# kfkq/DQMC

Hardware: AMD Instinct MI355X
Metric: MC sweeps/sec, 2D Hubbard N=256 Ltau=200 (higher is better)
Workload: dtype f64; 1 GPU; cfg3: 16x16 Hubbard U=8.0 beta=8.0 Ltau=200 n_stab=10 t=1 mu=-0.1; chains_per_gpu=1, n_chains_total=1, parallelism=independent chains, 1 gpu x 1 chain

## Files before the change

dqmc_amd/csrc/common.h:

```cpp
#pragma once

#include <hip/hip_runtime.h>
#include <cstdint>
#include <memory>
#include <string>

struct dqmc_engine;

namespace dq {

constexpr int WAVE = 64;

void set_error(const std::string& msg);
const char* get_error();

#define DQ_HIP(call)                                                                    \
    do {                                                                                \
        hipError_t _e = (call);                                                         \
        if (_e != hipSuccess) {                                                         \
            ::dq::set_error(std::string(#call) + ": " + hipGetErrorString(_e));         \
            return -2;                                              \
        }                                                                               \
    } while (0)

// ... 20 lines not shown

struct Mat {
    double* p = nullptr;
    long stride = 0;
    __host__ __device__ double* at(int c) const { return p + (long)c * stride; }
};
struct CMat {
    const double* p = nullptr;
    long stride = 0;
    CMat() = default;
    __host__ __device__ CMat(const double* p_, long s) : p(p_), stride(s) {}
    __host__ __device__ CMat(const Mat& m) : p(m.p), stride(m.stride) {}
    __host__ __device__ const double* at(int c) const { return p + (long)c * stride; }
};
using Vec = Mat;
using CVec = CMat;

struct GemmDesc {
    CMat A, B;
    Mat C;
    Mat CT{nullptr, 0};
    CVec rs, ks, cs;
    int n = 0;
    int transA = 0;
    int accumulate = 0;
};
int launch_gemm(const GemmDesc& g, int n_chains, hipStream_t s);

int launch_build_expv(const int8_t* fields, long f_stride, int nt, int n, const double* tab_expv ,
                      double* expv, double* invexpv, long v_stride, int n_chains, hipStream_t s);
int launch_split_d(CVec d, Vec dl_inv, Vec ds, double* logsum, int n, int n_chains, hipStream_t s);
int launch_split_d2(CVec d1, Vec dl1, Vec ds1, CVec d2, Vec dl2, Vec ds2, int n, int n_chains, hipStream_t s);
int launch_measure_equal_time(CMat G, double* out, long out_stride, int L1, int L2, int accumulate, int n_chains, hipStream_t s);
int launch_measure_unequal_time(const double* Gtt, const double* Gt0, const double* G0t, double* out, long out_stride, int L1, int L2, int nt,
                                int accumulate, int n_chains, hipStream_t s);
int launch_axpb_identity(CMat in, Mat out, double a, double b, int n, int n_chains, hipStream_t s);
int launch_copy(CMat in, Mat out, long count, int n_chains, hipStream_t s);
int launch_set_identity(Mat out, int n, int n_chains, hipStream_t s);
int launch_transpose_scale(CMat in, Mat out, CVec rs, int n, int n_chains, hipStream_t s);
int launch_max_abs_diff(CMat A, CMat B, double* err, long err_stride, int n, int n_chains, hipStream_t s);
int launch_add_scaled_cols(CMat A, CMat B, CVec cs, Mat C, int n, int n_chains, hipStream_t s);
int launch_scale_rows(CMat in, CVec rs, Mat out, int n, int n_chains, hipStream_t s);
struct DevStats { double acc_rate, max_err, sum_err, n_err; long long n_accepted, n_proposed; };
int launch_fold_stats(DevStats* st, const int* acc, long acc_stride, int n_slices, const double* err, long err_stride, int n_err,
                      int n, int nt, int n_chains, hipStream_t s);

struct QrWork {
    double* tau; long tau_stride;
    int* jpvt; long jpvt_stride;
    unsigned long long* sync = nullptr; long sync_stride = 0;
    int* abort_words = nullptr;
    int* info = nullptr;
    double* pw = nullptr; long pw_stride = 0;
    int* pivpos = nullptr; long pivpos_stride = 0;
};
long qr_panel_work_doubles(int n);
int launch_qr_panel(Mat A, Mat L, QrWork w, int n, int n_chains, hipStream_t s);
long qrcp_coop_sync_granules(int n);
int qrcp_coop_workgroups(int n, int n_chains);
enum class QrFamily { Panel, ColumnOwner, Cooperative, Streaming };
int launch_to_ldr(QrFamily f, Mat A, Mat L, Vec d, Mat R, QrWork w, int n, int n_chains, hipStream_t s);

int launch_lu_blocked(Mat A, int* perm, long perm_stride, int* rowpos, long rowpos_stride, double* logabsdet, int accumulate_logdet,
                      int* info, int n, int n_chains, hipStream_t s);
int launch_lu_solve(CMat LU, const int* perm, long perm_stride, Mat X, CVec dg, int mode, int n, int n_chains, hipStream_t s);

int launch_tri_solve(CMat R, const int* perm, long perm_stride, Mat X, CVec dg, double* scratch, long scratch_stride, int n, int n_chains, hipStream_t s);

int launch_gj_solve(Mat A, Mat B, Mat X, Mat SA, double* tinv, int* perm, long perm_stride, int* rowpos, long rowpos_stride,
                    double* logabsdet, int accumulate_logdet, int* info, int n, int n_chains, hipStream_t s);

struct UpdateTables {
    double rb[4][3];
    double delta[4][3];
    double ev[4];
    double iev[4];
    double pad[32];
};
struct UpdateDesc {
    Mat G;
    int8_t* fields; long f_stride;
    double* expv; double* invexpv; long v_stride;
    const UpdateTables* tabs;
    const int32_t* perm; const uint8_t* kprop; const double* u; long rs_stride;
    double* Upanel; double* Wpanel; long panel_stride;
    double* Cpanel = nullptr;
    int* state; long state_stride;
    double* prep; long prep_stride;
    Mat GT{nullptr, 0};
    int gt_valid = 0;
    void* slice_sync = nullptr;
    unsigned slice_epoch = 0;
    int slice_absent_tile = -1;
    int slice_absent_l = -1;
    int slice_late_tile = -1, slice_late_us = 0;
    int* info = nullptr;
    int* acc_out; long acc_stride;
    int n, nt;
};
constexpr int UPDATE_KD = 32;

struct SliceSync {
    unsigned long long seq; unsigned int error; unsigned int solo_count; unsigned int pad[12];
    unsigned int arrive[496];
};
constexpr size_t SLICE_SYNC_BYTES = 2048;
static_assert(sizeof(SliceSync) == SLICE_SYNC_BYTES, "SliceSync layout");
constexpr unsigned SLICE_EPOCH_LIMIT = 1u << 24;
constexpr unsigned SLICE_SOLO_BIT = 1u << 30, SLICE_FINAL_BIT = 1u << 31;
// ... 36 lines not shown
```

dqmc_amd/csrc/engine.hip:

```cpp
#include "common.h"
#include "../../include/dqmc_hip.h"

#include <cmath>
#include <cstdlib>
#include <cstring>
#include <map>
#include <memory>
#include <mutex>
#include <vector>

namespace dq {

static thread_local std::string g_err;
void set_error(const std::string& msg) { g_err = msg; }
const char* get_error() { return g_err.c_str(); }

int init_device_kernels(int device) {
    static std::mutex mu; static bool done[64] = {};
    std::lock_guard<std::mutex> lk(mu);
    if (device < 0 || device >= 64) { set_error("device ordinal out of range"); return -1; }
    if (done[device]) return 0;
    DQ_HIP(hipSetDevice(device));
    DQ_TRY(update_init_device()); DQ_TRY(update_sm_init_device()); DQ_TRY(qr_init_device()); DQ_TRY(qr_colown_init_device());
    done[device] = true;
    return 0;
}

struct Switches { bool qr_panel, qr_streaming, walk_submatrix, lu_classic, slice_multikernel; };
static const Switches& switches() {
    static const Switches sw = [] {
        const char* panel = getenv("DQMC_QR_PANEL");
        return Switches{!(panel && atoi(panel) == 0), getenv("DQMC_QR_STREAMING") != nullptr, getenv("DQMC_WALK_SUBMATRIX") != nullptr,
                        getenv("DQMC_LU_CLASSIC") != nullptr, getenv("DQMC_SLICE_MULTIKERNEL") != nullptr};
    }();
    return sw;
}

constexpr int GJ_MAX_N = 1024, GJ_MAX_CHAINS = 8;
constexpr int TRI_MAX_N = 640;

static QrFamily pick_qr(int n, int chains, bool allow_panel) {
    const Switches& sw = switches();
    if (sw.qr_streaming) return QrFamily::Streaming;
    if (allow_panel && sw.qr_panel && n >= 64 && n <= 1024 && n % 16 == 0 && chains <= 8) return QrFamily::Panel;
    if (n <= 256) return QrFamily::ColumnOwner;
    return qrcp_coop_workgroups(n, chains) <= 200 ? QrFamily::Cooperative : QrFamily::Streaming;
}

struct KernelPlan {
    QrFamily qr;
    enum class Solve { GaussJordan, BlockedLu } solve;
    enum class Rinv { Blocked, PerColumn } rinv;
    static KernelPlan pick(int n, int chains) {
        return KernelPlan{pick_qr(n, chains, true),
                          n <= GJ_MAX_N && chains <= GJ_MAX_CHAINS && !switches().lu_classic ? Solve::GaussJordan : Solve::BlockedLu,
                          n <= TRI_MAX_N ? Rinv::Blocked : Rinv::PerColumn};
    }
};

static SlicePath pick_slice_path(int n, int chains, bool reserved) {
    const Switches& sw = switches();
    const bool walk = n <= 256;
    if (sw.slice_multikernel) return SlicePath::Pairs;
    if (reserved) return walk && !sw.walk_submatrix ? SlicePath::PersistentWalk : SlicePath::PersistentSubmatrix;
    if (!walk) return SlicePath::Pairs;
    return chains >= 224 ? SlicePath::Solo : SlicePath::PairsTailSolo;
}
static bool is_persistent(SlicePath p) { return p == SlicePath::PersistentWalk || p == SlicePath::PersistentSubmatrix; }

struct LdrRef {
    Mat L; Vec d; Mat R;
    int* jpvt = nullptr;
    bool* tri = nullptr;
    Mat X{nullptr, 0};
    bool* xok = nullptr;
    void touch() const { if (xok) *xok = false; }
};
struct LdrStore {
    int n = 0, C = 0;
    DevPtr<double> L, d, R, X;
    DevPtr<int> jpvt;
    std::unique_ptr<bool[]> tri, xok;
    int alloc(int k, int n_, int C_, bool with_x = false) {
        n = n_; C = C_;
        const size_t nn = (size_t)n * n;
        DQ_TRY(dev_alloc(L, (size_t)k * C * nn)); DQ_TRY(dev_alloc(d, (size_t)k * C * n));
        DQ_TRY(dev_alloc(R, (size_t)k * C * nn)); DQ_TRY(dev_alloc(jpvt, (size_t)k * C * n));
        if (with_x) DQ_TRY(dev_alloc(X, (size_t)k * C * nn));
        tri.reset(new bool[k]()); xok.reset(new bool[k]());
        return 0;
    }
    LdrRef at(int i) const {
        const long nn = (long)n * n;
        LdrRef f{Mat{L.get() + (long)i * C * nn, nn}, Vec{d.get() + (long)i * C * n, (long)n}, Mat{R.get() + (long)i * C * nn, nn},
                 jpvt.get() + (long)i * C * n, &tri[i]};
        if (X) { f.X = Mat{X.get() + (long)i * C * nn, nn}; f.xok = &xok[i]; }
        return f;
    }
};

struct Ctx {
    int n = 0, C = 0, device = 0;
    long nn = 0;
    hipStream_t stream = nullptr;
    static constexpr int NT = 6, NV = 5;
    DevPtr<double> pool;
    DevPtr<double> vpool;
    DevPtr<int> ipool;
    DevPtr<unsigned long long> qsync;
    DevPtr<int> qabort;
    DevPtr<double> tinv;
    DevPtr<double> qpw;
    DevPtr<int> qpivpos;
    DevPtr<double> trinv;
    KernelPlan plan{};

    Mat T(int k) const { return Mat{pool.get() + (long)k * C * nn, nn}; }
    Vec V(int k) const { return Vec{vpool.get() + (long)k * C * n, (long)n}; }
    int* jpvt() const { return ipool.get(); }
    int* lperm() const { return ipool.get() + (long)C * n; }
    int* rowpos() const { return ipool.get() + 2L * C * n; }
    int* info() const { return ipool.get() + 3L * C * n; }

    int init(int n_, int C_, int device_) {
        n = n_; C = C_; device = device_; nn = (long)n * n;
        DQ_HIP(hipSetDevice(device));
        DQ_TRY(init_device_kernels(device));
        DQ_HIP(hipStreamCreateWithFlags(&stream, hipStreamNonBlocking));
        DQ_TRY(dev_alloc(pool, (size_t)NT * C * nn));
        DQ_TRY(dev_alloc(vpool, (size_t)NV * C * n));
        DQ_TRY(dev_alloc(ipool, 3L * C * n + 4));
        plan = KernelPlan::pick(n, C);
        if (plan.qr == QrFamily::Cooperative) { DQ_TRY(dev_alloc(qsync, (size_t)qrcp_coop_sync_granules(n) * C)); DQ_TRY(dev_alloc(qabort, C)); }
        if (plan.qr == QrFamily::Panel) { DQ_TRY(dev_alloc(qpw, (size_t)qr_panel_work_doubles(n) * C)); DQ_TRY(dev_alloc(qpivpos, (size_t)n * C)); }
        if (plan.solve == KernelPlan::Solve::GaussJordan) DQ_TRY(dev_alloc(tinv, (size_t)2048 * C));
        if (plan.rinv == KernelPlan::Rinv::Blocked) DQ_TRY(dev_alloc(trinv, (size_t)16 * (n + 16) * C));
        DQ_HIP(hipMemsetAsync(ipool.get(), 0, sizeof(int) * (3L * C * n + 4), stream));
        return 0;
    }
    ~Ctx() { if (stream) (void)hipStreamDestroy(stream); }

    int gemm(CMat A, CMat B, Mat Cm, CVec rs = CVec(), CVec ks = CVec(), CVec cs = CVec(), int transA = 0, int accumulate = 0, Mat CT = Mat{nullptr, 0}) {
        GemmDesc g; g.A = A; g.B = B; g.C = Cm; g.CT = CT; g.rs = rs; g.ks = ks; g.cs = cs; g.n = n; g.transA = transA; g.accumulate = accumulate;
        return launch_gemm(g, C, stream);
    }
    int to_ldr(Mat A, LdrRef out, bool direct = true) {
        const bool keep = direct && out.jpvt != nullptr;
        QrWork w{V(4).p, (long)n, keep ? out.jpvt : jpvt(), (long)n};
        w.sync = qsync.get(); w.sync_stride = qrcp_coop_sync_granules(n); w.abort_words = qabort.get(); w.info = info();
        w.pw = qpw.get(); w.pw_stride = qr_panel_work_doubles(n); w.pivpos = qpivpos.get(); w.pivpos_stride = n;
        if (out.tri) *out.tri = keep;
        out.touch();
        return launch_to_ldr(plan.qr, A, out.L, out.d, out.R, w, n, C, stream);
    }
    int r_inverse_scaled(LdrRef F, CVec dinv, Mat scratch, Mat lu_scratch, Mat* Xout) {
        const Mat X = F.X.p ? F.X : scratch;
        *Xout = X;
        if (F.xok && *F.xok) return 0;
        if (F.tri && *F.tri && F.jpvt) {
            if (plan.rinv == KernelPlan::Rinv::Blocked) DQ_TRY(launch_tri_solve(F.R, F.jpvt, n, X, dinv, trinv.get(), 16L * (n + 16), n, C, stream));
            else DQ_TRY(launch_lu_solve(F.R, F.jpvt, n, X, dinv, 2, n, C, stream));
        } else {
            DQ_TRY(launch_copy(F.R, lu_scratch, nn, C, stream));
            DQ_TRY(launch_lu_blocked(lu_scratch, lperm(), n, rowpos(), n, nullptr, 0, info(), n, C, stream));
            DQ_TRY(launch_lu_solve(lu_scratch, lperm(), n, X, dinv, 1, n, C, stream));
        }
        if (F.xok) *F.xok = true;
        return 0;
    }
    int mat_mul_ldr(CMat M, LdrRef F, LdrRef out) {
        DQ_TRY(gemm(M, F.L, T(0), CVec(), CVec(), CVec(F.d)));
        LdrRef q{out.L, out.d, T(1)};
        DQ_TRY(to_ldr(T(0), q));
        if (out.tri) *out.tri = false;
        out.touch();
        return gemm(T(1), F.R, out.R);
    }
    int ldr_mul_mat(LdrRef F, CMat M, LdrRef out) {
        DQ_TRY(gemm(F.R, M, T(0), CVec(F.d)));
        LdrRef q{T(1), out.d, out.R, out.jpvt, out.tri};
        q.xok = out.xok;
        DQ_TRY(to_ldr(T(0), q));
        return gemm(F.L, T(1), out.L);
    }
    int ldr_mul_ldr(LdrRef F1, LdrRef F2, LdrRef out) {
        DQ_TRY(gemm(F1.R, F2.L, T(0), CVec(F1.d), CVec(), CVec(F2.d)));
        LdrRef q{T(1), out.d, T(2)};
        DQ_TRY(to_ldr(T(0), q));
        if (out.tri) *out.tri = false;
        out.touch();
        DQ_TRY(gemm(F1.L, T(1), out.L));
        return gemm(T(2), F2.R, out.R);
    }
    int solve(Mat M, Mat RHS, Mat out, double* logdet_acc, Mat* Y) {
        if (plan.solve == KernelPlan::Solve::GaussJordan) {
            DQ_TRY(launch_gj_solve(M, RHS, out, T(5), tinv.get(), lperm(), n, rowpos(), n, logdet_acc, 1, info(), n, C, stream));
            *Y = out; return 0;
        }
        DQ_TRY(launch_lu_blocked(M, lperm(), n, rowpos(), n, logdet_acc, 1, info(), n, C, stream));
        DQ_TRY(launch_lu_solve(M, lperm(), n, RHS, CVec(), 0, n, C, stream));
        *Y = RHS; return 0;
    }
    int inv_I_plus_ldr(LdrRef F, Mat G, double* logdet ) {
// ... 972 lines not shown
```

dqmc_amd/csrc/qr_panel.hip:

```cpp
#include "common.h"
#include "wave.h"
#include <utility>

namespace dq {

namespace {

#ifdef DQ_QP_STAMPS
#define QST(i) { unsigned long long t_; asm volatile("s_memtime %0\n\ts_waitcnt lgkmcnt(0)" : "=s"(t_) :: "memory"); if (threadIdx.x == 0) qst[i] = t_; }
#else
#define QST(i)
#endif

constexpr int QP_B = 16;
constexpr int QP_SR = 32;
#ifndef QP_SEL_ROWS
#define QP_SEL_ROWS 32
#endif
constexpr int QP_SEL = QP_SEL_ROWS;
typedef double d4 __attribute__((ext_vector_type(4)));

__device__ __forceinline__ unsigned qp_row_bits(unsigned r) {
    unsigned h = r * 0x9E3779B1u + 0x85EBCA77u;
    h ^= h >> 16; h *= 0x85EBCA6Bu; h ^= h >> 13; h *= 0xC2B2AE35u; h ^= h >> 16;
// ... 140 lines not shown
            if ((blk_live >> b) & 1u) {
                double dlo0 = 0.0, dlo1 = 0.0, dhi0 = 0.0, dhi1 = 0.0;
#pragma unroll
                for (int i = 0; i < 16; ++i) {
                    if (i <= J) { if (i & 1) dpp_fmac_self<J>(dlo1, a[b][i]); else dpp_fmac_self<J>(dlo0, a[b][i]); }
                    else { if (i & 1) dpp_fmac_self<J>(dhi1, a[b][i]); else dpp_fmac_self<J>(dhi0, a[b][i]); }
                }
                acc += (dhi0 + dhi1) + (((diag >> b) & 1u) ? 0.0 : dlo0 + dlo1);
                if ((diag >> b) & 1u) sh.prow[par][c] = a[b][J];
            }
        }
        const double part = rows4_sum(acc);
        if (g == 0) sh.part[par][c][wave] = part;
    } else if (g == 0) sh.part[par][c][wave] = 0.0;
    lds_barrier();
    double s_c = sh.part[par][c][0], s_j = sh.part[par][J][0];
#pragma unroll
    for (int q = 1; q < NW; ++q) { s_c += sh.part[par][c][q]; s_j += sh.part[par][J][q]; }
    const double alpha = sh.prow[par][J], apc = sh.prow[par][c];
    double beta, tau, scale;
    householder<2>(alpha, s_j, beta, tau, scale);
    const double zc = fma(scale, s_c, apc);
    if (c == J) myscale = scale;
    if (blk_live) {
        const double mcf = c > J ? -scale * tau * zc : 0.0;
#pragma unroll
        for (int b = 0; b < CPL; ++b) {
            if ((blk_live >> b) & 1u) {
                const bool isd = (diag >> b) & 1u;
                const double mlo = isd ? 0.0 : mcf;
#pragma unroll
                for (int i = 0; i < 16; ++i) {
                    if (i <= J) dpp_axpy_self<J>(a[b][i], mlo);
                    else dpp_axpy_self<J>(a[b][i], mcf);
                }
                const double newd = c > J ? fma(-tau, zc, a[b][J]) : beta;
                a[b][J] = (isd && c >= J) ? newd : a[b][J];
                dpp_fence(a[b]);
            }
        }
    }
    if (wave == 0) {
        double zt = myscale * zc;
        double tj = 0.0;
        dpp_fence1(zt);
        t_row_dot(tj, trow, zt, std::make_integer_sequence<int, J>{});
        trow[J] = c < J ? -tau * tj : (c == J ? tau : 0.0);
        if (g == 0 && c == J) tau_out[J] = tau;
    }
}

}

template <int NW, int CPL>
__global__ __launch_bounds__(64 * NW) void qp_panel_kernel(Mat Am, QrWork w, int n, int k) {
    __shared__ PanelShared<NW> sh;
    const int chain = blockIdx.y;
    double* __restrict__ A = Am.at(chain);
    double* __restrict__ pw = w.pw + (long)chain * w.pw_stride;
    const double* __restrict__ Y = pw;
    double* __restrict__ Vp = pw + (long)QP_SR * n + (long)n * k;
    double* __restrict__ Tm = pw + (long)QP_SR * n + (long)n * n + (long)QP_B * k;
    double* __restrict__ VTp = pw + (long)QP_SR * n + (long)n * n + (long)QP_B * n + (long)n * k;
    int* __restrict__ pivpos = w.pivpos + (long)chain * w.pivpos_stride;
    double* tau = w.tau + (long)chain * w.tau_stride;
    int* jpvt = w.jpvt + (long)chain * w.jpvt_stride;
    const int t = threadIdx.x, lane = t & 63, wave = t >> 6;

#ifdef DQ_QP_STAMPS
    __shared__ unsigned long long qst[40];
#endif
    QST(0)
    {
        unsigned live = 0u;
        double y[CPL][QP_SEL]; int pp[CPL];
#pragma unroll
        for (int q = 0; q < CPL; ++q) {
            const int col = t + 64 * NW * q, cc = col < n ? col : n - 1;
#pragma unroll
            for (int i = 0; i < QP_SEL; ++i) y[q][i] = Y[(long)i * n + cc];
            pp[q] = pivpos[cc];
        }
#pragma unroll
        for (int q = 0; q < CPL; ++q) {
            const int col = t + 64 * NW * q;
            if (col < n && pp[q] < 0) live |= 1u << q;
            if (col >= n) {
#pragma unroll
                for (int i = 0; i < QP_SEL; ++i) y[q][i] = 0.0;
            }
        }
        if (y[0][0] == 1.2345e300) live = 0u;
        QST(1)
#define QP_SEL_STEP(J) select_step<J, NW, CPL>(y, live, t, lane, wave, sh); QST(2 + J)
        QP_SEL_STEP(0) QP_SEL_STEP(1) QP_SEL_STEP(2) QP_SEL_STEP(3) QP_SEL_STEP(4) QP_SEL_STEP(5) QP_SEL_STEP(6) QP_SEL_STEP(7)
        QP_SEL_STEP(8) QP_SEL_STEP(9) QP_SEL_STEP(10) QP_SEL_STEP(11) QP_SEL_STEP(12) QP_SEL_STEP(13) QP_SEL_STEP(14) QP_SEL_STEP(15)
#undef QP_SEL_STEP
    }
    lds_barrier();
    const int c = lane & 15, g = lane >> 4;
    const int mycol = sh.sel[c];
    double a[CPL][16], trow[QP_B], myscale = 0.0;
    unsigned diag = 0u, blk_live = 0u;
#pragma unroll
    for (int b = 0; b < CPL; ++b) {
        const int r0 = 64 * NW * b + 64 * wave + 16 * g;
        if (r0 == k) diag |= 1u << b;
        if (64 * NW * b + 64 * wave + 64 > k && 64 * NW * b + 64 * wave < n) blk_live |= 1u << b;
        const double2* src = reinterpret_cast<const double2*>(A + (long)n * mycol + r0);
        const bool rows_live = r0 >= k && r0 < n;
#pragma unroll
        for (int i = 0; i < 16; i += 2) { const double2 v = rows_live ? src[i >> 1] : double2{0.0, 0.0}; a[b][i] = v.x; a[b][i + 1] = v.y; }
        dpp_fence(a[b]);
    }
#pragma unroll
    for (int i = 0; i < QP_B; ++i) trow[i] = 0.0;
    double* tau_out = tau + k;
#ifdef DQ_QP_STAMPS
    if (a[0][0] == 1.2345e300) myscale = 1.0;
#endif
    QST(18)
#define QP_PAN(J) panel_step<J, NW, CPL>(a, trow, myscale, diag, blk_live, c, g, wave, sh, tau_out); QST(19 + J)
    QP_PAN(0) QP_PAN(1) QP_PAN(2) QP_PAN(3) QP_PAN(4) QP_PAN(5) QP_PAN(6) QP_PAN(7)
    QP_PAN(8) QP_PAN(9) QP_PAN(10) QP_PAN(11) QP_PAN(12) QP_PAN(13) QP_PAN(14) QP_PAN(15)
#undef QP_PAN
#pragma unroll
    for (int b = 0; b < CPL; ++b) {
        const int r0 = 64 * NW * b + 64 * wave + 16 * g;
        if (r0 >= k && r0 < n) {
            const bool isd = (diag >> b) & 1u;
            double2* dst = reinterpret_cast<double2*>(A + (long)n * mycol + r0);
            double2* vdst = reinterpret_cast<double2*>(Vp + (long)n * c + r0);
            double v[16], vc[16];
#pragma unroll
            for (int i = 0; i < 16; ++i) {
                const bool below = !isd || i > c;
                v[i] = below ? a[b][i] * myscale : a[b][i];
                vc[i] = below ? v[i] : (i == c ? 1.0 : 0.0);
                VTp[(long)QP_B * (r0 + i) + c] = vc[i];
            }
#pragma unroll
            for (int i = 0; i < 16; i += 2) { dst[i >> 1] = double2{v[i], v[i + 1]}; vdst[i >> 1] = double2{vc[i], vc[i + 1]}; }
        }
    }
    if (wave == 0 && g == 0) {
#pragma unroll
        for (int i = 0; i < QP_B; ++i) Tm[c + QP_B * i] = trow[i];
        jpvt[k + c] = mycol;
        pivpos[mycol] = k + c;
    }
#ifdef DQ_QP_STAMPS
    asm volatile("s_waitcnt vmcnt(0)" ::: "memory");
    QST(35)
    __syncthreads();
    if (t == 0 && k == 0 && blockIdx.y == 0) {
        printf("panel k=0 n=%d (100 MHz ticks x 24 = clk @2.4GHz): load Y %llu | sel steps", n, qst[1] - qst[0]);
        for (int j = 0; j < 16; ++j) printf(" %llu", qst[2 + j] - qst[1 + j]);
        printf(" | gather %llu | panel steps", qst[18] - qst[17]);
        for (int j = 0; j < 16; ++j) printf(" %llu", qst[19 + j] - qst[18 + j]);
        printf(" | write-out %llu | total %llu\n", qst[35] - qst[34], qst[35] - qst[0]);
    }
#endif
}

constexpr int QP_UW = 8;
constexpr int QP_YT = QP_SR / 16;

template <int TPW>
__device__ __forceinline__ void qp_q_role(double (&red)[QP_UW][QP_YT * 4][64], double* __restrict__ Qacc, double* __restrict__ L,
                                          const double* __restrict__ Vp, const double* __restrict__ VTp, const double* __restrict__ Tm,
                                          int n, int k, int cb) {
    const int t = threadIdx.x, lane = t & 63, wave = t >> 6;
    const int r16 = lane & 15, kk = lane >> 4;
    const int col = 16 * cb + r16;
    double* __restrict__ Qc = Qacc + (long)n * col;
    const int m_tiles = (n - k) / 16;
    d4 Qt[TPW]; double v1[TPW][4], v2[TPW][4], tv[4];
#pragma unroll
// ... 13 lines not shown
#pragma unroll
    for (int s = 0; s < 4; ++s) tv[s] = Tm[(kk + 4 * s) + QP_B * r16];
    const bool first = k == 0;
#pragma unroll
    for (int ti = 0; ti < TPW; ++ti)
#pragma unroll
        for (int r = 0; r < 4; ++r) Qt[ti][r] = first ? ((16 * (wave + QP_UW * ti) + kk + 4 * r == col) ? 1.0 : 0.0) : Qt[ti][r];
    d4 acc = {0.0, 0.0, 0.0, 0.0};
#pragma unroll
    for (int ti = 0; ti < TPW; ++ti) {
#pragma unroll
        for (int s = 0; s < 4; ++s) acc = __builtin_amdgcn_mfma_f64_16x16x4f64(v1[ti][s], Qt[ti][s], acc, 0, 0, 0);
    }
#pragma unroll
    for (int r = 0; r < 4; ++r) red[wave][r][lane] = acc[r];
    __syncthreads();
    d4 W;
#pragma unroll
    for (int r = 0; r < 4; ++r) {
        double v = red[0][r][lane];
#pragma unroll
        for (int q = 1; q < QP_UW; ++q) v += red[q][r][lane];
        W[r] = v;
    }
    d4 wp = {0.0, 0.0, 0.0, 0.0};
#pragma unroll
    for (int s = 0; s < 4; ++s) wp = __builtin_amdgcn_mfma_f64_16x16x4f64(tv[s], W[s], wp, 0, 0, 0);
    wp = -wp;
#pragma unroll
    for (int ti = 0; ti < TPW; ++ti) {
        const int rt = wave + QP_UW * ti;
        if (rt < m_tiles) {
            const int r0 = k + 16 * rt;
#pragma unroll
            for (int s = 0; s < 4; ++s) Qt[ti] = __builtin_amdgcn_mfma_f64_16x16x4f64(v2[ti][s], wp[s], Qt[ti], 0, 0, 0);
            if (rt == 0) {
#pragma unroll
                for (int r = 0; r < 4; ++r) L[(long)n * (k + kk + 4 * r) + col] = Qt[ti][r];
            } else {
#pragma unroll
                for (int r = 0; r < 4; ++r) Qc[r0 + kk + 4 * r] = Qt[ti][r];
            }
        }
    }
}

template <bool UPDATE, int TPW>
__global__ __launch_bounds__(64 * QP_UW) void qp_update_kernel(Mat Am, QrWork w, int n, int k, Mat Lm, int q_first) {
    constexpr int YT = QP_YT;
    __shared__ double red[QP_UW][YT * 4][64];
    const int chain = blockIdx.y;
    double* __restrict__ pw = w.pw + (long)chain * w.pw_stride;
    if (UPDATE && (int)blockIdx.x >= q_first) {
        qp_q_role<TPW>(red, pw + (long)(QP_SR + 2 * n) * n + (long)QP_B * n, Lm.at(chain), pw + (long)QP_SR * n + (long)n * k,
                       pw + (long)QP_SR * n + (long)n * n + (long)QP_B * n + (long)n * k, pw + (long)QP_SR * n + (long)n * n + (long)QP_B * k, n, k,
                       (int)blockIdx.x - q_first);
        return;
    }
    double* __restrict__ A = Am.at(chain);
    double* __restrict__ Y = pw;
    const double* __restrict__ Vp = pw + (long)QP_SR * n + (long)n * k;
    const double* __restrict__ Tm = pw + (long)QP_SR * n + (long)n * n + (long)QP_B * k;
    const double* __restrict__ VTp = pw + (long)QP_SR * n + (long)n * n + (long)QP_B * n + (long)n * k;
    int* __restrict__ pivpos = w.pivpos + (long)chain * w.pivpos_stride;
    const int t = threadIdx.x, lane = t & 63, wave = t >> 6;
    const int r16 = lane & 15, kk = lane >> 4;
    const int col = 16 * blockIdx.x + r16;
    double* __restrict__ Ac = A + (long)n * col;
    const int m_tiles = (n - k) / 16;
    int pp = -1;
    if (UPDATE) pp = pivpos[col];
    d4 At[TPW]; double v1[TPW][4], v2[TPW][4], tv[4];
#pragma unroll
    for (int ti = 0; ti < TPW; ++ti) {
        const int rt = wave + QP_UW * ti;
        At[ti] = d4{0.0, 0.0, 0.0, 0.0};
#pragma unroll
        for (int s = 0; s < 4; ++s) { v1[ti][s] = 0.0; v2[ti][s] = 0.0; }
        if (rt < m_tiles) {
            const int r0 = k + 16 * rt;
#pragma unroll
            for (int r = 0; r < 4; ++r) At[ti][r] = Ac[r0 + kk + 4 * r];
            if (UPDATE) {
#pragma unroll
                for (int s = 0; s < 4; ++s) { v1[ti][s] = VTp[(long)QP_B * (r0 + kk + 4 * s) + r16]; v2[ti][s] = Vp[(long)n * (kk + 4 * s) + (r0 + r16)]; }
            }
        }
    }
    if (UPDATE) {
#pragma unroll
        for (int s = 0; s < 4; ++s) tv[s] = Tm[(kk + 4 * s) + QP_B * r16];
    }
    const bool live_col = pp < 0;
    if (UPDATE) { if (__ballot(live_col) == 0ULL) return; }
    else if (t < 16) pivpos[col] = -1;
    d4 wp = {0.0, 0.0, 0.0, 0.0};
    if (UPDATE) {
        d4 acc = {0.0, 0.0, 0.0, 0.0};
#pragma unroll
        for (int ti = 0; ti < TPW; ++ti) {
#pragma unroll
            for (int s = 0; s < 4; ++s) acc = __builtin_amdgcn_mfma_f64_16x16x4f64(v1[ti][s], At[ti][s], acc, 0, 0, 0);
        }
#pragma unroll
        for (int r = 0; r < 4; ++r) red[wave][r][lane] = acc[r];
        __syncthreads();
        d4 W;
#pragma unroll
        for (int r = 0; r < 4; ++r) {
            double v = red[0][r][lane];
#pragma unroll
            for (int q = 1; q < QP_UW; ++q) v += red[q][r][lane];
            W[r] = live_col ? v : 0.0;
        }
#pragma unroll
        for (int s = 0; s < 4; ++s) wp = __builtin_amdgcn_mfma_f64_16x16x4f64(tv[s], W[s], wp, 0, 0, 0);
        wp = -wp;
        __syncthreads();
    }
    d4 ya[YT];
#pragma unroll
    for (int yt = 0; yt < YT; ++yt) ya[yt] = d4{0.0, 0.0, 0.0, 0.0};
#pragma unroll
    for (int ti = 0; ti < TPW; ++ti) {
        const int rt = wave + QP_UW * ti;
        if (rt < m_tiles) {
            const int r0 = k + 16 * rt;
            if (UPDATE) {
#pragma unroll
                for (int s = 0; s < 4; ++s) At[ti] = __builtin_amdgcn_mfma_f64_16x16x4f64(v2[ti][s], wp[s], At[ti], 0, 0, 0);
                if (live_col) {
#pragma unroll
                    for (int r = 0; r < 4; ++r) Ac[r0 + kk + 4 * r] = At[ti][r];
                }
            }
            if (!UPDATE || rt >= 1) {
#pragma unroll
                for (int s = 0; s < 4; ++s) {
                    const unsigned bits = qp_row_bits((unsigned)(r0 + kk + 4 * s));
#pragma unroll
                    for (int yt = 0; yt < YT; ++yt) ya[yt] = __builtin_amdgcn_mfma_f64_16x16x4f64(qp_sign(bits, 16 * yt + r16), At[ti][s], ya[yt], 0, 0, 0);
                }
            }
        }
    }
#pragma unroll
    for (int yt = 0; yt < YT; ++yt)
#pragma unroll
        for (int r = 0; r < 4; ++r) red[wave][4 * yt + r][lane] = ya[yt][r];
    __syncthreads();
    for (int idx = t; idx < YT * 4 * 64; idx += 64 * QP_UW) {
        const int l = idx & 63, q = idx >> 6, yt = q >> 2, r = q & 3;
        double v = red[0][q][l];
#pragma unroll
        for (int qq = 1; qq < QP_UW; ++qq) v += red[qq][q][l];
        Y[(long)(16 * yt + (l >> 4) + 4 * r) * n + 16 * blockIdx.x + (l & 15)] = v;
    }
}

static bool qr_panel_ok(int n, const QrWork& w) { return n >= 16 && n <= 1024 && n % 16 == 0 && w.pw != nullptr && w.pivpos != nullptr && w.pw_stride >= qr_panel_work_doubles(n); }
long qr_panel_work_doubles(int n) { return (long)(QP_SR + 3 * n) * n + (long)QP_B * n; }

int launch_qr_panel(Mat A, Mat L, QrWork w, int n, int n_chains, hipStream_t s) {
    if (!qr_panel_ok(n, w)) { set_error("panel QR: n must be a multiple of 16 in [16, 1024] and the workspace present"); return -1; }
    const int nb = n / 16;
    const int tpw = (nb + QP_UW - 1) / QP_UW;
#define QP_UPD(U, K, GRID, QFIRST) do { const dim3 ugrid(GRID, n_chains); \
                          if (tpw <= 2) hipLaunchKernelGGL((qp_update_kernel<U, 2>), ugrid, dim3(64 * QP_UW), 0, s, A, w, n, K, L, QFIRST); \
                          else if (tpw <= 5) hipLaunchKernelGGL((qp_update_kernel<U, 5>), ugrid, dim3(64 * QP_UW), 0, s, A, w, n, K, L, QFIRST); \
                          else hipLaunchKernelGGL((qp_update_kernel<U, 8>), ugrid, dim3(64 * QP_UW), 0, s, A, w, n, K, L, QFIRST); } while (0)
    QP_UPD(false, 0, nb, nb);
    for (int k = 0; k < n; k += QP_B) {
#define QP_LAUNCH(NW, CPL) hipLaunchKernelGGL((qp_panel_kernel<NW, CPL>), dim3(1, n_chains), dim3(64 * NW), 0, s, A, w, n, k)
        if (n <= 64) QP_LAUNCH(1, 1); else if (n <= 128) QP_LAUNCH(2, 1); else if (n <= 256) QP_LAUNCH(4, 1); else if (n <= 512) QP_LAUNCH(4, 2);
        else if (n <= 576) QP_LAUNCH(3, 3); else if (n <= 768) QP_LAUNCH(4, 3); else QP_LAUNCH(4, 4);
#undef QP_LAUNCH
        if (k + QP_B < n) QP_UPD(true, k, 2 * nb, nb);
        else QP_UPD(true, k, nb, 0);
    }
#undef QP_UPD
    DQ_HIP(hipGetLastError());
    return 0;
}

}
```

Before: 12.81 sweeps/s.

## Fuse QR panel factorization and trailing update into one per-step kernel

Replaces the two launches per panel step (a single-workgroup panel factorization, then the update kernel) with one fused step kernel. Every workgroup redundantly factors the panel in LDS and takes an atomic ticket, and the last arriver writes back the pivot, tau and diagonal data. The pivot-selection sketch Y is double-buffered by step parity, and a smaller workspace layout is used for the fused path. This removes a launch and a global round-trip for V and T at each step, at the cost of redundant panel work in every block and reliance on cross-workgroup ordering through the ticket counter.

```diff
diff --git a/dqmc_amd/csrc/common.h b/dqmc_amd/csrc/common.h
--- a/dqmc_amd/csrc/common.h
+++ b/dqmc_amd/csrc/common.h
@@ -96,9 +96,12 @@
     int* abort_words = nullptr;
     int* info = nullptr;
     double* pw = nullptr; long pw_stride = 0;
+    bool pw_two_launch = false;
     int* pivpos = nullptr; long pivpos_stride = 0;
 };
-long qr_panel_work_doubles(int n);
+bool qr_panel_fused_fits(int n);
+bool qr_panel_fused_default(int n);
+long qr_panel_work_doubles(int n, bool two_launch);
 int launch_qr_panel(Mat A, Mat L, QrWork w, int n, int n_chains, hipStream_t s);
 long qrcp_coop_sync_granules(int n);
 int qrcp_coop_workgroups(int n, int n_chains);
diff --git a/dqmc_amd/csrc/engine.hip b/dqmc_amd/csrc/engine.hip
--- a/dqmc_amd/csrc/engine.hip
+++ b/dqmc_amd/csrc/engine.hip
@@ -26,11 +26,12 @@
     return 0;
 }
 
-struct Switches { bool qr_panel, qr_streaming, walk_submatrix, lu_classic, slice_multikernel; };
+struct Switches { bool qr_panel; int qr_panel_fused; bool qr_streaming, walk_submatrix, lu_classic, slice_multikernel; };
 static const Switches& switches() {
     static const Switches sw = [] {
         const char* panel = getenv("DQMC_QR_PANEL");
-        return Switches{!(panel && atoi(panel) == 0), getenv("DQMC_QR_STREAMING") != nullptr, getenv("DQMC_WALK_SUBMATRIX") != nullptr,
+        const char* fused = getenv("DQMC_QR_PANEL_FUSED");
+        return Switches{!(panel && atoi(panel) == 0), fused ? (atoi(fused) != 0 ? 1 : 0) : -1, getenv("DQMC_QR_STREAMING") != nullptr, getenv("DQMC_WALK_SUBMATRIX") != nullptr,
                         getenv("DQMC_LU_CLASSIC") != nullptr, getenv("DQMC_SLICE_MULTIKERNEL") != nullptr};
     }();
     return sw;
@@ -111,6 +112,7 @@
     DevPtr<int> qabort;
     DevPtr<double> tinv;
     DevPtr<double> qpw;
+    bool qpw_two_launch = false;
     DevPtr<int> qpivpos;
     DevPtr<double> trinv;
     KernelPlan plan{};
@@ -132,7 +134,13 @@
         DQ_TRY(dev_alloc(ipool, 3L * C * n + 4));
         plan = KernelPlan::pick(n, C);
         if (plan.qr == QrFamily::Cooperative) { DQ_TRY(dev_alloc(qsync, (size_t)qrcp_coop_sync_granules(n) * C)); DQ_TRY(dev_alloc(qabort, C)); }
-        if (plan.qr == QrFamily::Panel) { DQ_TRY(dev_alloc(qpw, (size_t)qr_panel_work_doubles(n) * C)); DQ_TRY(dev_alloc(qpivpos, (size_t)n * C)); }
+        if (plan.qr == QrFamily::Panel) {
+            const int fused = switches().qr_panel_fused;
+            qpw_two_launch = !(fused < 0 ? qr_panel_fused_default(n) : fused == 1 && qr_panel_fused_fits(n));
+            const size_t qpw_count = (size_t)qr_panel_work_doubles(n, qpw_two_launch) * C;
+            DQ_TRY(dev_alloc(qpw, qpw_count)); DQ_TRY(dev_alloc(qpivpos, (size_t)n * C));
+            DQ_HIP(hipMemsetAsync(qpw.get(), 0, sizeof(double) * qpw_count, stream));
+        }
         if (plan.solve == KernelPlan::Solve::GaussJordan) DQ_TRY(dev_alloc(tinv, (size_t)2048 * C));
         if (plan.rinv == KernelPlan::Rinv::Blocked) DQ_TRY(dev_alloc(trinv, (size_t)16 * (n + 16) * C));
         DQ_HIP(hipMemsetAsync(ipool.get(), 0, sizeof(int) * (3L * C * n + 4), stream));
@@ -148,7 +156,7 @@
         const bool keep = direct && out.jpvt != nullptr;
         QrWork w{V(4).p, (long)n, keep ? out.jpvt : jpvt(), (long)n};
         w.sync = qsync.get(); w.sync_stride = qrcp_coop_sync_granules(n); w.abort_words = qabort.get(); w.info = info();
-        w.pw = qpw.get(); w.pw_stride = qr_panel_work_doubles(n); w.pivpos = qpivpos.get(); w.pivpos_stride = n;
+        w.pw = qpw.get(); w.pw_stride = qr_panel_work_doubles(n, qpw_two_launch); w.pw_two_launch = qpw_two_launch; w.pivpos = qpivpos.get(); w.pivpos_stride = n;
         if (out.tri) *out.tri = keep;
         out.touch();
         return launch_to_ldr(plan.qr, A, out.L, out.d, out.R, w, n, C, stream);
diff --git a/dqmc_amd/csrc/qr_panel.hip b/dqmc_amd/csrc/qr_panel.hip
--- a/dqmc_amd/csrc/qr_panel.hip
+++ b/dqmc_amd/csrc/qr_panel.hip
@@ -216,6 +216,85 @@
 
 }
 
+__host__ __device__ __forceinline__ long qp_off_qacc(int n) { return 2L * QP_SR * n; }
+__host__ __device__ __forceinline__ long qp_off_ticket(int n) { return qp_off_qacc(n) + (long)n * n; }
+__host__ __device__ __forceinline__ long qp_off_vp(int n) { return qp_off_ticket(n) + 2; }
+__host__ __device__ __forceinline__ long qp_off_tm(int n) { return qp_off_vp(n) + (long)n * n; }
+__host__ __device__ __forceinline__ long qp_off_vtp(int n) { return qp_off_tm(n) + (long)QP_B * n; }
+
+#ifdef DQ_QP_STAMPS
+#define QP_QST_PARAM , unsigned long long* qst
+#define QP_QST_ARG , qst
+#else
+#define QP_QST_PARAM
+#define QP_QST_ARG
+#endif
+
+template <int NW, int CPL, class Pre, class Mid>
+__device__ __forceinline__ bool qp_factor_panel(const double* A, const double* __restrict__ Y, const int* pivpos, int n, int k, PanelShared<NW>& sh,
+                                                double* tau_out, double (&a)[CPL][16], double (&trow)[QP_B], double& myscale, unsigned& diag, int& mycol,
+                                                Pre&& pre, Mid&& mid QP_QST_PARAM) {
+    const int t = threadIdx.x, lane = t & 63, wave = t >> 6;
+    QST(0)
+    {
+        unsigned live = 0u;
+        double y[CPL][QP_SEL]; int pp[CPL];
+#pragma unroll
+        for (int q = 0; q < CPL; ++q) {
+            const int col = t + 64 * NW * q, cc = col < n ? col : n - 1;
+#pragma unroll
+            for (int i = 0; i < QP_SEL; ++i) y[q][i] = Y[(long)i * n + cc];
+            pp[q] = pivpos[cc];
+        }
+        if (pre()) return false;
+#pragma unroll
+        for (int q = 0; q < CPL; ++q) {
+            const int col = t + 64 * NW * q;
+            if (col < n && pp[q] < 0) live |= 1u << q;
+            if (col >= n) {
+#pragma unroll
+                for (int i = 0; i < QP_SEL; ++i) y[q][i] = 0.0;
+            }
+        }
+        if (y[0][0] == 1.2345e300) live = 0u;
+        QST(1)
+#define QP_SEL_STEP(J) select_step<J, NW, CPL>(y, live, t, lane, wave, sh); QST(2 + J)
+        QP_SEL_STEP(0) QP_SEL_STEP(1) QP_SEL_STEP(2) QP_SEL_STEP(3) QP_SEL_STEP(4) QP_SEL_STEP(5) QP_SEL_STEP(6) QP_SEL_STEP(7)
+        QP_SEL_STEP(8) QP_SEL_STEP(9) QP_SEL_STEP(10) QP_SEL_STEP(11) QP_SEL_STEP(12) QP_SEL_STEP(13) QP_SEL_STEP(14) QP_SEL_STEP(15)
+#undef QP_SEL_STEP
+    }
+    lds_barrier();
+    const int c = lane & 15, g = lane >> 4;
+    mycol = sh.sel[c];
+    myscale = 0.0; diag = 0u;
+    unsigned blk_live = 0u;
+#pragma unroll
+    for (int b = 0; b < CPL; ++b) {
+        const int r0 = 64 * NW * b + 64 * wave + 16 * g;
+        if (r0 == k) diag |= 1u << b;
+        if (64 * NW * b + 64 * wave + 64 > k && 64 * NW * b + 64 * wave < n) blk_live |= 1u << b;
+        const double2* src = reinterpret_cast<const double2*>(A + (long)n * mycol + r0);
+        const bool rows_live = r0 >= k && r0 < n;
+#pragma unroll
+        for (int i = 0; i < 16; i += 2) { const double2 v = rows_live ? src[i >> 1] : double2{0.0, 0.0}; a[b][i] = v.x; a[b][i + 1] = v.y; }
+        dpp_fence(a[b]);
+    }
+    asm volatile("s_waitcnt vmcnt(0)" ::: "memory");
+#pragma unroll
+    for (int i = 0; i < QP_B; ++i) trow[i] = 0.0;
+#ifdef DQ_QP_STAMPS
+    if (a[0][0] == 1.2345e300) myscale = 1.0;
+#endif
+    QST(18)
+#define QP_PAN(J) panel_step<J, NW, CPL>(a, trow, myscale, diag, blk_live, c, g, wave, sh, tau_out); QST(19 + J)
+    QP_PAN(0)
+    mid();
+    QP_PAN(1) QP_PAN(2) QP_PAN(3) QP_PAN(4) QP_PAN(5) QP_PAN(6) QP_PAN(7)
+    QP_PAN(8) QP_PAN(9) QP_PAN(10) QP_PAN(11) QP_PAN(12) QP_PAN(13) QP_PAN(14) QP_PAN(15)
+#undef QP_PAN
+    return true;
+}
+
 template <int NW, int CPL>
 __global__ __launch_bounds__(64 * NW) void qp_panel_kernel(Mat Am, QrWork w, int n, int k) {
     __shared__ PanelShared<NW> sh;
@@ -223,71 +302,21 @@
     double* __restrict__ A = Am.at(chain);
     double* __restrict__ pw = w.pw + (long)chain * w.pw_stride;
     const double* __restrict__ Y = pw;
-    double* __restrict__ Vp = pw + (long)QP_SR * n + (long)n * k;
-    double* __restrict__ Tm = pw + (long)QP_SR * n + (long)n * n + (long)QP_B * k;
-    double* __restrict__ VTp = pw + (long)QP_SR * n + (long)n * n + (long)QP_B * n + (long)n * k;
+    double* __restrict__ Vp = pw + qp_off_vp(n) + (long)n * k;
+    double* __restrict__ Tm = pw + qp_off_tm(n) + (long)QP_B * k;
+    double* __restrict__ VTp = pw + qp_off_vtp(n) + (long)n * k;
     int* __restrict__ pivpos = w.pivpos + (long)chain * w.pivpos_stride;
     double* tau = w.tau + (long)chain * w.tau_stride;
     int* jpvt = w.jpvt + (long)chain * w.jpvt_stride;
     const int t = threadIdx.x, lane = t & 63, wave = t >> 6;
+    const int c = lane & 15, g = lane >> 4;
 
 #ifdef DQ_QP_STAMPS
     __shared__ unsigned long long qst[40];
 #endif
-    QST(0)
-    {
-        unsigned live = 0u;
-        double y[CPL][QP_SEL]; int pp[CPL];
-#pragma unroll
-        for (int q = 0; q < CPL; ++q) {
-            const int col = t + 64 * NW * q, cc = col < n ? col : n - 1;
-#pragma unroll
-            for (int i = 0; i < QP_SEL; ++i) y[q][i] = Y[(long)i * n + cc];
-            pp[q] = pivpos[cc];
-        }
-#pragma unroll
-        for (int q = 0; q < CPL; ++q) {
-            const int col = t + 64 * NW * q;
-            if (col < n && pp[q] < 0) live |= 1u << q;
-            if (col >= n) {
-#pragma unroll
-                for (int i = 0; i < QP_SEL; ++i) y[q][i] = 0.0;
-            }
-        }
-        if (y[0][0] == 1.2345e300) live = 0u;
-        QST(1)
-#define QP_SEL_STEP(J) select_step<J, NW, CPL>(y, live, t, lane, wave, sh); QST(2 + J)
-        QP_SEL_STEP(0) QP_SEL_STEP(1) QP_SEL_STEP(2) QP_SEL_STEP(3) QP_SEL_STEP(4) QP_SEL_STEP(5) QP_SEL_STEP(6) QP_SEL_STEP(7)
-        QP_SEL_STEP(8) QP_SEL_STEP(9) QP_SEL_STEP(10) QP_SEL_STEP(11) QP_SEL_STEP(12) QP_SEL_STEP(13) QP_SEL_STEP(14) QP_SEL_STEP(15)
-#undef QP_SEL_STEP
-    }
-    lds_barrier();
-    const int c = lane & 15, g = lane >> 4;
-    const int mycol = sh.sel[c];
-    double a[CPL][16], trow[QP_B], myscale = 0.0;
-    unsigned diag = 0u, blk_live = 0u;
-#pragma unroll
-    for (int b = 0; b < CPL; ++b) {
-        const int r0 = 64 * NW * b + 64 * wave + 16 * g;
-        if (r0 == k) diag |= 1u << b;
-        if (64 * NW * b + 64 * wave + 64 > k && 64 * NW * b + 64 * wave < n) blk_live |= 1u << b;
-        const double2* src = reinterpret_cast<const double2*>(A + (long)n * mycol + r0);
-        const bool rows_live = r0 >= k && r0 < n;
-#pragma unroll
-        for (int i = 0; i < 16; i += 2) { const double2 v = rows_live ? src[i >> 1] : double2{0.0, 0.0}; a[b][i] = v.x; a[b][i + 1] = v.y; }
-        dpp_fence(a[b]);
-    }
-#pragma unroll
-    for (int i = 0; i < QP_B; ++i) trow[i] = 0.0;
-    double* tau_out = tau + k;
-#ifdef DQ_QP_STAMPS
-    if (a[0][0] == 1.2345e300) myscale = 1.0;
-#endif
-    QST(18)
-#define QP_PAN(J) panel_step<J, NW, CPL>(a, trow, myscale, diag, blk_live, c, g, wave, sh, tau_out); QST(19 + J)
-    QP_PAN(0) QP_PAN(1) QP_PAN(2) QP_PAN(3) QP_PAN(4) QP_PAN(5) QP_PAN(6) QP_PAN(7)
-    QP_PAN(8) QP_PAN(9) QP_PAN(10) QP_PAN(11) QP_PAN(12) QP_PAN(13) QP_PAN(14) QP_PAN(15)
-#undef QP_PAN
+    double a[CPL][16], trow[QP_B], myscale;
+    unsigned diag; int mycol;
+    qp_factor_panel<NW, CPL>(A, Y, pivpos, n, k, sh, tau + k, a, trow, myscale, diag, mycol, [] { return false; }, [] {} QP_QST_ARG);
 #pragma unroll
     for (int b = 0; b < CPL; ++b) {
         const int r0 = 64 * NW * b + 64 * wave + 16 * g;
@@ -407,16 +436,15 @@
     const int chain = blockIdx.y;
     double* __restrict__ pw = w.pw + (long)chain * w.pw_stride;
     if (UPDATE && (int)blockIdx.x >= q_first) {
-        qp_q_role<TPW>(red, pw + (long)(QP_SR + 2 * n) * n + (long)QP_B * n, Lm.at(chain), pw + (long)QP_SR * n + (long)n * k,
-                       pw + (long)QP_SR * n + (long)n * n + (long)QP_B * n + (long)n * k, pw + (long)QP_SR * n + (long)n * n + (long)QP_B * k, n, k,
-                       (int)blockIdx.x - q_first);
+        qp_q_role<TPW>(red, pw + qp_off_qacc(n), Lm.at(chain), pw + qp_off_vp(n) + (long)n * k, pw + qp_off_vtp(n) + (long)n * k,
+                       pw + qp_off_tm(n) + (long)QP_B * k, n, k, (int)blockIdx.x - q_first);
         return;
     }
     double* __restrict__ A = Am.at(chain);
     double* __restrict__ Y = pw;
-    const double* __restrict__ Vp = pw + (long)QP_SR * n + (long)n * k;
-    const double* __restrict__ Tm = pw + (long)QP_SR * n + (long)n * n + (long)QP_B * k;
-    const double* __restrict__ VTp = pw + (long)QP_SR * n + (long)n * n + (long)QP_B * n + (long)n * k;
+    const double* __restrict__ Vp = pw + qp_off_vp(n) + (long)n * k;
+    const double* __restrict__ Tm = pw + qp_off_tm(n) + (long)QP_B * k;
+    const double* __restrict__ VTp = pw + qp_off_vtp(n) + (long)n * k;
     int* __restrict__ pivpos = w.pivpos + (long)chain * w.pivpos_stride;
     const int t = threadIdx.x, lane = t & 63, wave = t >> 6;
     const int r16 = lane & 15, kk = lane >> 4;
@@ -513,11 +541,232 @@
     }
 }
 
-static bool qr_panel_ok(int n, const QrWork& w) { return n >= 16 && n <= 1024 && n % 16 == 0 && w.pw != nullptr && w.pivpos != nullptr && w.pw_stride >= qr_panel_work_doubles(n); }
-long qr_panel_work_doubles(int n) { return (long)(QP_SR + 3 * n) * n + (long)QP_B * n; }
+template <int NW, int CPL, int TPW>
+__global__ __launch_bounds__(64 * NW) void qp_step_kernel(Mat Am, QrWork w, int n, int k, Mat Lm, int q_first) {
+    constexpr int YT = QP_YT;
+    constexpr int NV = (QP_UW + NW - 1) / NW;
+    constexpr int LDV = 64 * NW * CPL + 1;
+    __shared__ PanelShared<NW> sh;
+    __shared__ double Vs[QP_B * LDV];
+    __shared__ double Ts[QP_B * (QP_B + 1)];
+    __shared__ double red[QP_UW][YT * 4][64];
+    __shared__ double s_tau[QP_B];
+    __shared__ unsigned s_ticket;
+#ifdef DQ_QP_STAMPS
+    __shared__ unsigned long long qst[40];
+#endif
+    const int chain = blockIdx.y;
+    double* pw = w.pw + (long)chain * w.pw_stride;
+    const bool qrole = (int)blockIdx.x >= q_first;
+    const int cb = qrole ? (int)blockIdx.x - q_first : (int)blockIdx.x;
+    double* A = Am.at(chain);
+    const int par = (k / QP_B) & 1;
+    const double* __restrict__ Yr = pw + (long)par * QP_SR * n;
+    double* __restrict__ Yw = pw + (long)(par ^ 1) * QP_SR * n;
+    unsigned* counter = reinterpret_cast<unsigned*>(pw + qp_off_ticket(n));
+    int* pivpos = w.pivpos + (long)chain * w.pivpos_stride;
+    const int t = threadIdx.x, lane = t & 63, wave = t >> 6;
+    const int r16 = lane & 15, kk = lane >> 4;
+    const int col = 16 * cb + r16;
+    double* Xc = (qrole ? pw + qp_off_qacc(n) : A) + (long)n * col;
+    const int m_tiles = (n - k) / 16;
+    const int pp_ld = pivpos[col];
+    d4 X[NV][TPW];
+#pragma unroll
+    for (int vi = 0; vi < NV; ++vi) {
+#pragma unroll
+        for (int ti = 0; ti < TPW; ++ti) {
+            const int vw = wave + NW * vi, rt = vw + QP_UW * ti;
+            X[vi][ti] = d4{0.0, 0.0, 0.0, 0.0};
+            if (vw < QP_UW && rt < m_tiles) {
+#pragma unroll
+                for (int r = 0; r < 4; ++r) X[vi][ti][r] = Xc[k + 16 * rt + kk + 4 * r];
+            }
+        }
+    }
+    const int pp = qrole ? -1 : pp_ld;
+    const unsigned last_ticket = gridDim.x - 1;
+    bool have_ticket = false;
+    unsigned ticket = 0u;
+    double a[CPL][16], trow[QP_B], myscale;
+    unsigned diag; int mycol;
+    const bool factored = qp_factor_panel<NW, CPL>(A, Yr, pivpos, n, k, sh, s_tau, a, trow, myscale, diag, mycol, [&] {
+        if (__ballot(pp < 0) != 0ULL) return false;
+        if (t == 0) s_ticket = __hip_atomic_fetch_add(counter, 1u, __ATOMIC_RELAXED, __HIP_MEMORY_SCOPE_AGENT);
+        __syncthreads();
+        have_ticket = true;
+        return s_ticket != last_ticket;
+    }, [&] {
+        if (!have_ticket && t == 0) {
+            long off = 0;
+            asm volatile("" : "+v"(off));
+            ticket = __hip_atomic_fetch_add(counter + off, 1u, __ATOMIC_RELAXED, __HIP_MEMORY_SCOPE_AGENT);
+        }
+    } QP_QST_ARG);
+    if (!factored) return;
+    const int c = lane & 15, g = lane >> 4;
+#pragma unroll
+    for (int b = 0; b < CPL; ++b) {
+        const int r0 = 64 * NW * b + 64 * wave + 16 * g;
+        if (r0 >= k && r0 < n) {
+            const bool isd = (diag >> b) & 1u;
+#pragma unroll
+            for (int i = 0; i < 16; ++i) {
+                const bool below = !isd || i > c;
+                Vs[c * LDV + r0 + i] = below ? a[b][i] * myscale : (i == c ? 1.0 : 0.0);
+            }
+        }
+    }
+    if (wave == 0 && g == 0) {
+#pragma unroll
+        for (int i = 0; i < QP_B; ++i) Ts[c + (QP_B + 1) * i] = trow[i];
+    }
+    if (!have_ticket && t == 0) s_ticket = ticket;
+    __syncthreads();
+    QST(35)
+    if (s_ticket == last_ticket) {
+        double* tau = w.tau + (long)chain * w.tau_stride;
+        int* jpvt = w.jpvt + (long)chain * w.jpvt_stride;
+#pragma unroll
+        for (int b = 0; b < CPL; ++b) {
+            if ((diag >> b) & 1u) {
+#pragma unroll
+                for (int i = 0; i < 16; ++i) if (i <= c) A[(long)n * mycol + k + i] = a[b][i];
+            }
+        }
+        if (wave == 0 && g == 0) { jpvt[k + c] = mycol; pivpos[mycol] = k + c; tau[k + c] = s_tau[c]; }
+        if (t == 0) *counter = 0u;
+        if (have_ticket) return;
+    }
+    QST(36)
+    bool sel_hit = false;
+#pragma unroll
+    for (int j = 0; j < QP_B; ++j) sel_hit |= sh.sel[j] == col;
+    const bool live_col = qrole || (pp < 0 && !sel_hit);
+    double tv[4];
+#pragma unroll
+    for (int s = 0; s < 4; ++s) tv[s] = Ts[(kk + 4 * s) + (QP_B + 1) * r16];
+    const bool first = qrole && k == 0;
+#pragma unroll
+    for (int vi = 0; vi < NV; ++vi)
+#pragma unroll
+        for (int ti = 0; ti < TPW; ++ti)
+#pragma unroll
+            for (int r = 0; r < 4; ++r) X[vi][ti][r] = first ? ((16 * (wave + NW * vi + QP_UW * ti) + kk + 4 * r == col) ? 1.0 : 0.0) : X[vi][ti][r];
+#pragma unroll
+    for (int vi = 0; vi < NV; ++vi) {
+        const int vw = wave + NW * vi;
+        if (vw < QP_UW) {
+            d4 acc = {0.0, 0.0, 0.0, 0.0};
+#pragma unroll
+            for (int ti = 0; ti < TPW; ++ti) {
+                const int rt = vw + QP_UW * ti;
+                if (rt < m_tiles) {
+                    const double* vrow = Vs + r16 * LDV + (k + 16 * rt + kk);
+#pragma unroll
+                    for (int s = 0; s < 4; ++s) acc = __builtin_amdgcn_mfma_f64_16x16x4f64(vrow[4 * s], X[vi][ti][s], acc, 0, 0, 0);
+                }
+            }
+#pragma unroll
+            for (int r = 0; r < 4; ++r) red[vw][r][lane] = acc[r];
+        }
+    }
+    __syncthreads();
+    d4 W;
+#pragma unroll
+    for (int r = 0; r < 4; ++r) {
+        double v = red[0][r][lane];
+#pragma unroll
+        for (int q = 1; q < QP_UW; ++q) v += red[q][r][lane];
+        W[r] = live_col ? v : 0.0;
+    }
+    d4 wp = {0.0, 0.0, 0.0, 0.0};
+#pragma unroll
+    for (int s = 0; s < 4; ++s) wp = __builtin_amdgcn_mfma_f64_16x16x4f64(tv[s], W[s], wp, 0, 0, 0);
+    wp = -wp;
+    __syncthreads();
+    QST(37)
+    double* L = Lm.at(chain);
+#pragma unroll
+    for (int vi = 0; vi < NV; ++vi) {
+        const int vw = wave + NW * vi;
+        if (vw < QP_UW) {
+            d4 ya[YT];
+#pragma unroll
+            for (int yt = 0; yt < YT; ++yt) ya[yt] = d4{0.0, 0.0, 0.0, 0.0};
+#pragma unroll
+            for (int ti = 0; ti < TPW; ++ti) {
+                const int rt = vw + QP_UW * ti;
+                if (rt < m_tiles) {
+                    const int r0 = k + 16 * rt;
+#pragma unroll
+                    for (int s = 0; s < 4; ++s) X[vi][ti] = __builtin_amdgcn_mfma_f64_16x16x4f64(Vs[(kk + 4 * s) * LDV + r0 + r16], wp[s], X[vi][ti], 0, 0, 0);
+                    if (qrole) {
+                        if (rt == 0) {
+#pragma unroll
+                            for (int r = 0; r < 4; ++r) L[(long)n * (k + kk + 4 * r) + col] = X[vi][ti][r];
+                        } else {
+#pragma unroll
+                            for (int r = 0; r < 4; ++r) Xc[r0 + kk + 4 * r] = X[vi][ti][r];
+                        }
+                    } else {
+                        if (live_col) {
+#pragma unroll
+                            for (int r = 0; r < 4; ++r) Xc[r0 + kk + 4 * r] = X[vi][ti][r];
+                        }
+                        if (rt >= 1) {
+#pragma unroll
+                            for (int s = 0; s < 4; ++s) {
+                                const unsigned bits = qp_row_bits((unsigned)(r0 + kk + 4 * s));
+#pragma unroll
+                                for (int yt = 0; yt < YT; ++yt) ya[yt] = __builtin_amdgcn_mfma_f64_16x16x4f64(qp_sign(bits, 16 * yt + r16), X[vi][ti][s], ya[yt], 0, 0, 0);
+                            }
+                        }
+                    }
+                }
+            }
+            if (!qrole) {
+#pragma unroll
+                for (int yt = 0; yt < YT; ++yt)
+#pragma unroll
+                    for (int r = 0; r < 4; ++r) red[vw][4 * yt + r][lane] = ya[yt][r];
+            }
+        }
+    }
+    if (qrole) return;
+    __syncthreads();
+    for (int idx = t; idx < YT * 4 * 64; idx += 64 * NW) {
+        const int l = idx & 63, q = idx >> 6, yt = q >> 2, r = q & 3;
+        double v = red[0][q][l];
+#pragma unroll
+        for (int qq = 1; qq < QP_UW; ++qq) v += red[qq][q][l];
+        Yw[(long)(16 * yt + (l >> 4) + 4 * r) * n + 16 * cb + (l & 15)] = v;
+    }
+#ifdef DQ_QP_STAMPS
+    asm volatile("s_waitcnt vmcnt(0)" ::: "memory");
+    QST(38)
+    __syncthreads();
+    if (t == 0 && (k == 0 || k == n / 2) && blockIdx.x == 0 && blockIdx.y == 0) {
+        printf("step k=%d n=%d (100 MHz ticks): loads %llu | sel steps", k, n, qst[1] - qst[0]);
+        for (int j = 0; j < 16; ++j) printf(" %llu", qst[2 + j] - qst[1 + j]);
+        printf(" | gather %llu | panel steps", qst[18] - qst[17]);
+        for (int j = 0; j < 16; ++j) printf(" %llu", qst[19 + j] - qst[18 + j]);
+        printf(" | deposit + ticket %llu | last arriver %llu | W %llu | update + sketch %llu | total %llu\n", qst[35] - qst[34], qst[36] - qst[35],
+               qst[37] - qst[36], qst[38] - qst[37], qst[38] - qst[0]);
+    }
+#endif
+}
+
+bool qr_panel_fused_fits(int n) { return n <= 576; }
+bool qr_panel_fused_default(int n) { return n <= 512; }
+long qr_panel_work_doubles(int n, bool two_launch) { return two_launch ? qp_off_vtp(n) + (long)n * n : qp_off_vp(n); }
+static bool qr_panel_ok(int n, const QrWork& w, bool two_launch) {
+    return n >= 16 && n <= 1024 && n % 16 == 0 && w.pw != nullptr && w.pivpos != nullptr && w.pw_stride >= qr_panel_work_doubles(n, two_launch);
+}
 
 int launch_qr_panel(Mat A, Mat L, QrWork w, int n, int n_chains, hipStream_t s) {
-    if (!qr_panel_ok(n, w)) { set_error("panel QR: n must be a multiple of 16 in [16, 1024] and the workspace present"); return -1; }
+    const bool fused = !w.pw_two_launch && qr_panel_fused_fits(n);
+    if (!qr_panel_ok(n, w, !fused)) { set_error("panel QR: n must be a multiple of 16 in [16, 1024] and the workspace present"); return -1; }
     const int nb = n / 16;
     const int tpw = (nb + QP_UW - 1) / QP_UW;
 #define QP_UPD(U, K, GRID, QFIRST) do { const dim3 ugrid(GRID, n_chains); \
@@ -526,12 +775,20 @@
                           else hipLaunchKernelGGL((qp_update_kernel<U, 8>), ugrid, dim3(64 * QP_UW), 0, s, A, w, n, K, L, QFIRST); } while (0)
     QP_UPD(false, 0, nb, nb);
     for (int k = 0; k < n; k += QP_B) {
+        const bool trailing = k + QP_B < n;
+        const int grid = trailing ? 2 * nb : nb, q_first = trailing ? nb : 0;
+        if (fused) {
+#define QP_STEP(NW, CPL, TPW) hipLaunchKernelGGL((qp_step_kernel<NW, CPL, TPW>), dim3(grid, n_chains), dim3(64 * NW), 0, s, A, w, n, k, L, q_first)
+            if (n <= 64) QP_STEP(1, 1, 1); else if (n <= 128) QP_STEP(2, 1, 1); else if (n <= 256) QP_STEP(4, 1, 2); else if (n <= 512) QP_STEP(4, 2, 4);
+            else QP_STEP(3, 3, 5);
+#undef QP_STEP
+            continue;
+        }
 #define QP_LAUNCH(NW, CPL) hipLaunchKernelGGL((qp_panel_kernel<NW, CPL>), dim3(1, n_chains), dim3(64 * NW), 0, s, A, w, n, k)
         if (n <= 64) QP_LAUNCH(1, 1); else if (n <= 128) QP_LAUNCH(2, 1); else if (n <= 256) QP_LAUNCH(4, 1); else if (n <= 512) QP_LAUNCH(4, 2);
         else if (n <= 576) QP_LAUNCH(3, 3); else if (n <= 768) QP_LAUNCH(4, 3); else QP_LAUNCH(4, 4);
 #undef QP_LAUNCH
-        if (k + QP_B < n) QP_UPD(true, k, 2 * nb, nb);
-        else QP_UPD(true, k, nb, 0);
+        QP_UPD(true, k, grid, q_first);
     }
 #undef QP_UPD
     DQ_HIP(hipGetLastError());
```

After: 13.04 sweeps/s, median of 6. 1.02x the previous value.
